# StephenTaf/Modern-Search-Engines-Project

Measured on AMD Instinct MI355X. Metric: queries/sec, two-stage retrieval top-100 (BM25 top-1000 + dense full scan + rerank/fuse), higher is better.
Workload: dtype f32 (exact f32 cosines of every returned document; candidates filtered by one pass of f16 products with a measured margin; batches <= 64 queries: f16x2-split products, |err| <= 8e-6) (dense cosine) / f64 (BM25, fuse)

## Files before the change

modern-search-engines-project_amd/csrc/msr_bm25.hip:

```cpp
#include <stdio.h>

#include "msr_common.h"
#include "msr_internal.h"

namespace {

constexpr int BM25_TILE = MSR_BM25_TILE;
#ifndef BM25_WPW
#define BM25_WPW 1
#endif
constexpr int BM25_WAVES = BM25_WPW;
constexpr int BM25_THREADS = 64 * BM25_WAVES;
constexpr int BM25_TPW = 8;
constexpr int BM25_MAX_TERMS = 64;
constexpr int BM25_CAP = MSR_BM25_ROUND_CAP;
constexpr int BM25_RES = 4;
#ifndef BM25_U
#define BM25_U 4
#endif
#ifndef BM25_UM
#define BM25_UM 8
#endif
constexpr int BM25_WORDS = BM25_TPW * BM25_TILE / 32;
static_assert(BM25_WORDS == 4 * 64, "four bitmap words per lane");
static_assert(BM25_CAP % 128 == 0 && BM25_CAP >= 128 && BM25_CAP <= BM25_TILE, "whole batches of slots; a word (32) always fits");

__device__ __forceinline__ void lds_phase() {
    __builtin_amdgcn_fence(__ATOMIC_ACQ_REL, "wavefront");
    __builtin_amdgcn_wave_barrier();
}

__device__ __forceinline__ int64_t lane_i64(int64_t v, int j) {
    const uint32_t lo = (uint32_t)__builtin_amdgcn_readlane((int)(uint32_t)(uint64_t)v, j);
    const uint32_t hi = (uint32_t)__builtin_amdgcn_readlane((int)(uint32_t)((uint64_t)v >> 32), j);
    return (int64_t)(((uint64_t)hi << 32) | lo);
}
__device__ __forceinline__ double lane_f64(double v, int j) {
    return __longlong_as_double(lane_i64(__double_as_longlong(v), j));
}
__device__ __forceinline__ int lane_rank(unsigned long long m) {
    return (int)__builtin_amdgcn_mbcnt_hi((uint32_t)(m >> 32), __builtin_amdgcn_mbcnt_lo((uint32_t)m, 0u));
}

__device__ __forceinline__ double post_comp(const Bm25Post& x) { return __hiloint2double((int)x.comp_hi, (int)x.comp_lo); }
typedef const __attribute__((address_space(1))) double* gtable;
__device__ __forceinline__ gtable table_of(int64_t bits) { return (gtable)(uint64_t)bits; }

enum : int { K_DEAD = 0, K_LOOKUP = 1, K_HEAVY = 2, K_RANGE = 3 };

#ifndef BM25_WPE
#define BM25_WPE 4
#endif
template <typename... Set>
__global__ __launch_bounds__(BM25_THREADS) __attribute__((amdgpu_waves_per_eu(BM25_WPE, BM25_WPE))) void bm25_taat_kernel(Bm25Index ix,
                                                                  const int32_t* __restrict__ q_term_off,
                                                                  const int32_t* __restrict__ q_terms,
                                                                  const int32_t* __restrict__ q_qtf,
                                                                  int q_first, int nq, double min_score, int tpw, int n_spans,
                                                                  double* __restrict__ cand_score,
                                                                  int32_t* __restrict__ cand_doc,
                                                                  int32_t* __restrict__ seg_n, int dbg_arg, Set... set) {
#ifdef MSR_DIAG
    const int dbg = dbg_arg;
#else
    constexpr int dbg = 0;
#endif
    __shared__ __attribute__((aligned(16))) double acc_all[BM25_WAVES][BM25_CAP];
    __shared__ __attribute__((aligned(16))) uint32_t bits_all[BM25_WAVES][BM25_WORDS];
    __shared__ uint16_t pre_all[BM25_WAVES][BM25_WORDS];
    __shared__ uint16_t slot_all[BM25_WAVES][BM25_CAP];
    const int tid = threadIdx.x, lane = tid & 63;
    const int wave = __builtin_amdgcn_readfirstlane(tid >> 6);
    const int item = (int)blockIdx.x * BM25_WAVES + wave;
    const int span = item / nq, q = item - span * nq;
    if (span >= n_spans) return;
    int32_t* seg_len = seg_n + (int64_t)q * n_spans + span;
    int seg_cnt = 0;
    constexpr bool WITHIN = sizeof...(Set) > 0;
    MsrSetRow srow{nullptr, 0};
    if constexpr (WITHIN) {
        srow = msr_set_row(q_first + q, set...);
        if (srow.mode == 2) {
            if (lane == 0) *seg_len = 0;
            return;
        }
    }
    const int tile0 = span * tpw;
    const int n_my = tile0 + tpw <= ix.n_tiles ? tpw : ix.n_tiles - tile0;
    double* acc = acc_all[wave];
    uint32_t* bits = bits_all[wave];
    uint16_t* pre = pre_all[wave];
    uint16_t* slot = slot_all[wave];
    const int64_t lo_span = (int64_t)tile0 * BM25_TILE;
    const int64_t hi_span = lo_span + (int64_t)n_my * BM25_TILE < ix.n_docs ? lo_span + (int64_t)n_my * BM25_TILE : ix.n_docs;
    const uint32_t n_span = (uint32_t)(hi_span - lo_span);
    const bool prune = min_score >= 0.0 && ix.dense_id != nullptr && !(dbg & 64);
    int nt = 0, klass = K_DEAD;
    int64_t s_v = 0;
    int h_v = -1;
    int64_t ps_v = 0, pe_v = 0;
    double idf_v = 0.0, qtf_v = 0.0;
    bool medium = false;
    {
        const int t0 = q_term_off[q_first + q];
        nt = q_term_off[q_first + q + 1] - t0;
        if (nt > BM25_MAX_TERMS) nt = BM25_MAX_TERMS;
        if (lane < nt) {
            const int32_t t = q_terms[t0 + lane];
            if (t >= 0 && t < ix.n_terms) {
                const int64_t s = ix.term_off[t], e = ix.term_off[t + 1];
                if (e > s) {
                    idf_v = (double)ix.idf[t];
                    qtf_v = (double)q_qtf[t0 + lane];
                    const int dh = prune ? ix.dense_id[t] : -1;
                    const int h = ix.heavy_id ? ix.heavy_id[t] : -1;
                    if (dh >= 0 && idf_v < 0.0 && qtf_v > 0.0) {
                        klass = K_LOOKUP;
                        s_v = (int64_t)(ix.dense_comp + (int64_t)dh * ix.dense_stride);
                    } else if (h >= 0) {
                        klass = K_HEAVY;
                        s_v = s;
                        h_v = h;
                        const uint32_t* row = ix.tile_off + (int64_t)h * (ix.n_tiles + 1) + tile0;
                        ps_v = s + row[0];
                        pe_v = s + row[n_my];
                    } else {
                        klass = K_RANGE;
                        ps_v = s;
                        pe_v = e;
                        medium = e - s > 64;
                    }
                }
            }
        }
    }
    const unsigned long long look_mask = __ballot(klass == K_LOOKUP);
    const unsigned long long stream_mask = __ballot(klass >= K_HEAVY);
    if (stream_mask == 0) {
        if (lane == 0) *seg_len = 0;
        return;
    }
    const int64_t seg_base = (int64_t)q * ix.n_docs + lo_span;
    {
        const int64_t lo8 = lo_span, hi8 = hi_span;
        constexpr int MED = 4;
        unsigned long long todo = __ballot(medium);
        while (todo) {
            int jj[MED];
            int64_t s_[MED], e_[MED], ch_[MED];
            int32_t probe[MED];
#pragma unroll
            for (int m = 0; m < MED; ++m) {
                jj[m] = todo ? __ffsll((long long)todo) - 1 : -1;
                if (todo) todo &= todo - 1;
                probe[m] = 0; s_[m] = e_[m] = ch_[m] = 0;
                if (jj[m] >= 0) {
                    s_[m] = lane_i64(ps_v, jj[m]);
                    e_[m] = lane_i64(pe_v, jj[m]);
                    ch_[m] = (e_[m] - s_[m] + 63) >> 6;
                    int64_t idx = s_[m] + (int64_t)(lane + 1) * ch_[m] - 1;
                    if (idx > e_[m] - 1) idx = e_[m] - 1;
                    probe[m] = ix.post[idx].doc;
                }
            }
#pragma unroll
            for (int m = 0; m < MED; ++m) {
                if (jj[m] < 0) continue;
                const unsigned long long ge_lo = __ballot((int64_t)probe[m] >= lo8);
                const unsigned long long ge_hi = __ballot((int64_t)probe[m] >= hi8);
                int64_t ps = e_[m], pe = e_[m];
                if (ge_lo) {
                    ps = s_[m] + (int64_t)(__ffsll((long long)ge_lo) - 1) * ch_[m];
                    if (ps > e_[m]) ps = e_[m];
                    if (ge_hi) {
                        pe = s_[m] + (int64_t)(__ffsll((long long)ge_hi)) * ch_[m];
                        if (pe > e_[m]) pe = e_[m];
                    }
                }
                if (lane == jj[m]) { ps_v = ps; pe_v = pe; }
            }
        }
    }
    const int64_t null_post = ix.n_postings;
    int cj[BM25_RES];
    int64_t cps[BM25_RES], cpe[BM25_RES];
// ... 320 lines not shown
    }
}

__global__ __launch_bounds__(256) void bm25_dnorm_kernel(const int32_t* __restrict__ doc_len, int64_t n_docs, int64_t n_pad,
                                                          double k1, double b, double avgdl, double* __restrict__ out) {
    const int64_t i = (int64_t)blockIdx.x * 256 + threadIdx.x;
    if (i >= n_pad) return;
    const double omb = 1.0 - b;
    out[i] = i < n_docs ? k1 * (omb + (b * (double)doc_len[i]) / avgdl) : 1.0;
}

int g_bm25_dbg = 0;

}

void msr_bm25_set_dbg(int v) { g_bm25_dbg = v; }
hipError_t msr_bm25_build_skip(const Bm25Index& ix, const int32_t* heavy_terms, int n_heavy, uint32_t* tile_off,
                               hipStream_t stream) {
    if (n_heavy <= 0) return hipSuccess;
    build_skip_kernel<<<n_heavy, 256, 0, stream>>>(ix, heavy_terms, tile_off);
    return hipGetLastError();
}

hipError_t msr_bm25_post_comp(const int32_t* post_doc, const int32_t* post_tf, const double* dnorm, double k1, int64_t n,
                              Bm25Post* out, hipStream_t stream) {
    if (n < 0) return hipSuccess;
    bm25_post_comp_kernel<<<4096, 256, 0, stream>>>(post_doc, post_tf, dnorm, k1 + 1.0, n, out);
    return hipGetLastError();
}

hipError_t msr_bm25_build_dense(const Bm25Index& ix, const int32_t* dense_terms, int n_dense, double* dense_comp,
                                int64_t dense_stride, hipStream_t stream) {
    if (n_dense <= 0) return hipSuccess;
    bm25_dense_kernel<<<dim3(256, (unsigned)n_dense), 256, 0, stream>>>(ix, dense_terms, dense_comp, dense_stride);
    return hipGetLastError();
}

hipError_t msr_bm25_dnorm(const int32_t* doc_len, int64_t n_docs, int64_t n_pad, double k1, double b, double avgdl, double* out,
                          hipStream_t stream) {
    if (n_pad <= 0) return hipSuccess;
    bm25_dnorm_kernel<<<(unsigned)((n_pad + 255) / 256), 256, 0, stream>>>(doc_len, n_docs, n_pad, k1, b, avgdl, out);
    return hipGetLastError();
}

hipError_t msr_bm25_validate(const Bm25Index& ix, int32_t* flag, hipStream_t stream) {
    hipError_t err = hipMemsetAsync(flag, 0x7F, sizeof(int32_t), stream);
    if (err != hipSuccess) return err;
    validate_postings_kernel<<<2048, 256, 0, stream>>>(ix, flag);
    return hipGetLastError();
}

int msr_bm25_max_segments(int64_t n_docs) { return (int)((n_docs + BM25_TILE - 1) / BM25_TILE); }

__global__ __launch_bounds__(256) void bm25_window_kernel(Bm25Index ix, const int32_t* __restrict__ q_term_off,
                                                           const int32_t* __restrict__ q_terms,
                                                           const int32_t* __restrict__ q_qtf, int q_first, int nq,
                                                           uint64_t* __restrict__ out) {
    const int q = blockIdx.x * 256 + threadIdx.x;
    if (q >= nq) return;
    const int t0 = q_term_off[q_first + q];
    int nt = q_term_off[q_first + q + 1] - t0;
    if (nt > BM25_MAX_TERMS) nt = BM25_MAX_TERMS;
    double u = 0.0;
    for (int j = 0; j < nt; ++j) {
        const int32_t t = q_terms[t0 + j];
        if (t < 0 || t >= ix.n_terms) continue;
        const double w = (double)ix.idf[t] * (double)q_qtf[t0 + j];
        if (w > 0.0) u += w;
    }
    u = u * (ix.k1 + 1.0) * 1.0000001 + 1e-300;
    const uint64_t pre = msr_ord64(u) >> 44;
    out[q] = pre > 4094 ? pre - 4094 : 0;
}

hipError_t msr_bm25_window(const Bm25Index& ix, const int32_t* q_term_off, const int32_t* q_terms, const int32_t* q_qtf,
                           int q_first, int nq, uint64_t* out, hipStream_t stream) {
    if (nq <= 0) return hipSuccess;
    bm25_window_kernel<<<(unsigned)((nq + 255) / 256), 256, 0, stream>>>(ix, q_term_off, q_terms, q_qtf, q_first, nq, out);
    return hipGetLastError();
}

void msr_bm25_split(int n_tiles, int nq, int* tpw_out, int* n_spans_out) {
    int tpw = BM25_TPW;
    while (tpw > 1 && (int64_t)nq * ((n_tiles + tpw - 1) / tpw) < 8192) tpw >>= 1;
    *tpw_out = tpw;
    *n_spans_out = (n_tiles + tpw - 1) / tpw;
}

hipError_t msr_bm25_scores(const Bm25Index& ix, const int32_t* q_term_off, const int32_t* q_terms,
                           const int32_t* q_qtf, int q_first, int nq, double min_score, double* cand_score,
                           int32_t* cand_doc, int32_t* seg_n, int* n_seg, int64_t* seg_stride, hipStream_t stream,
                           const MsrSetView* set) {
    *n_seg = 0; *seg_stride = 0;
    if (nq <= 0 || ix.n_docs <= 0) return hipSuccess;
    int tpw = 1, n_spans = 0;
    msr_bm25_split(ix.n_tiles, nq, &tpw, &n_spans);
    const int64_t items = (int64_t)nq * n_spans;
    if (items >= (1ll << 31)) return hipErrorInvalidValue;
    *n_seg = n_spans;
    *seg_stride = (int64_t)tpw * BM25_TILE;
    const unsigned blocks = (unsigned)((items + BM25_WAVES - 1) / BM25_WAVES);
    if (set)
        bm25_taat_kernel<<<blocks, BM25_THREADS, 0, stream>>>(ix, q_term_off, q_terms, q_qtf, q_first, nq, min_score, tpw, n_spans,
                                                              cand_score, cand_doc, seg_n, g_bm25_dbg, *set);
    else
        bm25_taat_kernel<<<blocks, BM25_THREADS, 0, stream>>>(ix, q_term_off, q_terms, q_qtf, q_first, nq, min_score, tpw, n_spans,
                                                              cand_score, cand_doc, seg_n, g_bm25_dbg);
    return hipGetLastError();
}
```

modern-search-engines-project_amd/csrc/msr_engine.hip:

```cpp
#include <hip/hip_runtime.h>
#include <stdarg.h>
#include <stdio.h>
#include <stdlib.h>
#include <string.h>

#include <algorithm>
#include <new>
#include <vector>

#include "../../include/msretr.h"
#include "msr_devmem.h"
#include "msr_internal.h"

struct HipMem {
    static hipError_t alloc(void** p, size_t bytes) { return hipMalloc(p, bytes); }
    static void free(void* p) { (void)hipFree(p); }
};
using Group = DevGroup<HipMem>;

struct msr_engine {
    msr_config cfg;
    char err[512];
    Group mem_engine;
    Group mem_corpus;
    Group mem_postings;
    Group mem_chunks;
    Group mem_bf16;
    Bm25Index bm25{};
    bool have_postings = false;
    const int64_t* tok_off = nullptr;
    const int32_t* tok_ids = nullptr;
    int64_t n_tokens = 0;
    bool have_tokens = false;
    const int64_t* voc_char_off = nullptr;
    const uint16_t* voc_chars = nullptr;
    const uint32_t* voc_weight = nullptr;
    int64_t voc_n_chars = 0;
    bool have_vocab = false;
    FacetTable facet{};
    bool have_facet = false;
    const uint32_t* sig = nullptr;
    int64_t sig_n = 0;
    DenseIndex dense{};
    bool have_chunks = false;
    const int32_t* url_group = nullptr;
    int64_t url_group_n = 0;
    const int32_t* doc_domain = nullptr;
    int64_t doc_domain_n = 0;
    int32_t* chunk_doc = nullptr;
    void* emb_presplit = nullptr;
    void* row_meta = nullptr;
    float* inv_norm_own = nullptr;
    int32_t* span_doc = nullptr;
    int32_t* wspan_doc = nullptr;
    int32_t* wspan12_doc = nullptr;
    float* qn = nullptr;
    float* rr_qn = nullptr;
    void* qimg = nullptr;
    SelScratch sel{};
    float* rerank_cos = nullptr;
    int32_t* rerank_meta = nullptr;
    void* score_rows = nullptr;
    size_t score_rows_bytes = 0;
    int32_t* bm_cand_doc = nullptr;
    size_t bm_cand_bytes = 0;
    int32_t* bm_heavy_id = nullptr;
    void* bm_post = nullptr;
    int32_t* bm_dense_id = nullptr;
    double* bm_dense = nullptr;
    uint32_t* bm_tile_off = nullptr;
    int32_t* bm_cand_n = nullptr;
    uint64_t* bm_win = nullptr;
    uint64_t* voc_sig = nullptr;
    int32_t* bt_top_doc = nullptr; float* bt_top_score = nullptr; int32_t* bt_top_n = nullptr;
    int32_t* bt_cand_doc = nullptr; float* bt_cand_score = nullptr; int32_t* bt_cand_chunk = nullptr;
    int32_t* bt_cand_n = nullptr;
    int32_t* tile_row = nullptr;
    int n_tiles = 0;
    bool tiles_ok = false;
    GemmF32Index gf{};
    bool gf_ok = false;
    float* gf_inv_pad = nullptr; float* gf_qn = nullptr; void* gf_fb_qimg = nullptr;
    int32_t* gf_gate = nullptr;
    void* gf_emb_tiled = nullptr;
    void* gf_emb_f16 = nullptr;
    int32_t* tile_trow = nullptr;
    void* emb_bf16 = nullptr;
    GemmIndex gemm{};
    bool gemm_ok = false;
    float* gm_qn = nullptr;
    uint32_t* bf_err = nullptr;
    float* bf_margin = nullptr;
    float* bf_ones = nullptr;
    void* bf_row_meta = nullptr;
    DenseIndex dense_bf16{};
    int n_cus = 256;
    int split_pending = 0;
    int row_copy_state = 0;
    int row_image_state = 0;
    int last_dense_width = 0;
    int last_dense_segments = 0;
    int32_t* sim_flag = nullptr;
    void* sim_lists = nullptr; size_t sim_lists_bytes = 0;
    void* sim_over = nullptr; size_t sim_over_bytes = 0;
    bool timing = false;
    static constexpr int EV_RING = 256;
    static constexpr int EV_KINDS = 4;
    hipEvent_t ev_start[EV_KINDS][EV_RING] = {};
    hipEvent_t ev_stop[EV_KINDS][EV_RING] = {};
    int ev_count[EV_KINDS] = {0, 0, 0, 0};
};

static constexpr size_t GF_GATE_BYTES = 16 * sizeof(int32_t);

static thread_local char g_create_err[512] = "";

static int fail(msr_engine* e, int code, const char* fmt, ...) {
    char* dst = e ? e->err : g_create_err;
    va_list ap;
    va_start(ap, fmt);
    vsnprintf(dst, 512, fmt, ap);
    va_end(ap);
    return code;
}

// ... 116 lines not shown
    if (cfg->scan_variant != 0 && cfg->scan_variant != 2 && cfg->scan_variant != 7 && cfg->scan_variant != 14 &&
        cfg->scan_variant != 15)
        return fail(nullptr, MSR_ERR_INVALID, "msr_create: scan_variant must be 0, 2, 7, 14 or 15");
    if (cfg->flags & ~(int32_t)(MSR_CFG_NO_ROW_COPY | MSR_CFG_SINGLE_EMIT))
        return fail(nullptr, MSR_ERR_INVALID, "msr_create: unknown flag bits 0x%x", cfg->flags);
    int ndev = 0;
    hipError_t herr = hipGetDeviceCount(&ndev);
    if (herr != hipSuccess || ndev <= 0)
        return fail(nullptr, MSR_ERR_HIP, "msr_create: no HIP device available (%s)",
                    herr == hipSuccess ? "device count is 0" : hipGetErrorString(herr));
    if (cfg->device < 0 || cfg->device >= ndev)
        return fail(nullptr, MSR_ERR_INVALID, "msr_create: device %d out of range (have %d)", cfg->device, ndev);
    msr_engine* e = new (std::nothrow) msr_engine();
    if (!e) return fail(nullptr, MSR_ERR_NOMEM, "msr_create: out of host memory");
    e->cfg = *cfg;
    e->err[0] = 0;
    const int rc = create_scratch(e);
    if (rc) {
        fail(nullptr, rc, "msr_create: %s", e->err);
        msr_destroy(e);
        return rc;
    }
    *out = e;
    return MSR_OK;
}

extern "C" int msr_destroy(msr_engine* e) {
    if (!e) return MSR_OK;
    drop_postings(e);
    drop_chunks(e);
    for (int w = 0; w < msr_engine::EV_KINDS; ++w)
        for (int j = 0; j < msr_engine::EV_RING; ++j) {
            if (e->ev_start[w][j]) (void)hipEventDestroy(e->ev_start[w][j]);
            if (e->ev_stop[w][j]) (void)hipEventDestroy(e->ev_stop[w][j]);
        }
    delete e;
    return MSR_OK;
}

static int ensure_score_rows(msr_engine* e, int64_t n_docs) {
    const size_t pad = (size_t)(n_docs + 31) / 32 * 32;
    const size_t need = std::max((size_t)e->cfg.max_queries * pad * sizeof(double), (size_t)128 * pad * sizeof(float));
    return grow(e, e->mem_corpus, &e->score_rows, &e->score_rows_bytes, need, "score rows");
}

static int build_postings(msr_engine* e, Bm25Index cand, hipStream_t st) {
    const int64_t n_terms = cand.n_terms, n_postings = cand.n_postings, n_docs = cand.n_docs;
    int rc = ensure_score_rows(e, n_docs);
    if (rc) return rc;
    rc = grow(e, e->mem_corpus, &e->bm_cand_doc, &e->bm_cand_bytes, (size_t)e->cfg.max_queries * (size_t)n_docs * sizeof(int32_t),
              "BM25 candidate lists");
    if (rc) return rc;
    ALLOC(e, e->mem_postings, e->bm_win, (size_t)e->cfg.max_queries * sizeof(uint64_t));
    ALLOC(e, e->mem_postings, e->bm_cand_n, (size_t)e->cfg.max_queries * msr_bm25_max_segments(n_docs) * sizeof(int32_t));
    int32_t h_flag = 0;
    HIP_TRY(e, msr_bm25_validate(cand, e->sel.cand_n, st));
    HIP_TRY(e, hipMemcpyAsync(&h_flag, e->sel.cand_n, sizeof(int32_t), hipMemcpyDeviceToHost, st));
    HIP_TRY(e, hipMemsetAsync(e->sel.cand_n, 0, sizeof(int32_t), st));
    HIP_TRY(e, hipStreamSynchronize(st));
    if (h_flag >= 1 && h_flag <= 5) {
        static const char* why[] = {"", "term_off is not a monotone offset array ending at n_postings",
                                    "a posting's document index is outside [0, n_docs)",
                                    "documents are not strictly ascending inside a posting list",
                                    "negative doc_len", "non-positive term frequency"};
        return fail(e, MSR_ERR_INVALID, "msr_bind_postings: malformed index: %s", why[h_flag]);
    }
    if (!(cand.avgdl > 0.0) || !(cand.k1 >= 0.0) || !(cand.b >= 0.0 && cand.b <= 1.0))
        return fail(e, MSR_ERR_INVALID, "msr_bind_postings: avgdl must be > 0, k1 >= 0, 0 <= b <= 1");
    std::vector<int32_t> dense_terms;
    if (n_terms > 0) {
        std::vector<int64_t> h_toff((size_t)n_terms + 1);
        std::vector<float> h_idf((size_t)n_terms);
        HIP_TRY(e, hipMemcpyAsync(h_toff.data(), cand.term_off, h_toff.size() * sizeof(int64_t), hipMemcpyDeviceToHost, st));
        HIP_TRY(e, hipMemcpyAsync(h_idf.data(), cand.idf, h_idf.size() * sizeof(float), hipMemcpyDeviceToHost, st));
        HIP_TRY(e, hipStreamSynchronize(st));
        std::vector<int32_t> heavy_id((size_t)n_terms, -1), heavy_terms;
        for (int64_t t = 0; t < n_terms; ++t)
            if (h_toff[t + 1] - h_toff[t] >= MSR_BM25_HEAVY_DF && h_toff[t + 1] - h_toff[t] < (1ll << 32)) {
                heavy_id[t] = (int32_t)heavy_terms.size();
                heavy_terms.push_back((int32_t)t);
                if (h_idf[t] < 0.0f) dense_terms.push_back((int32_t)t);
            }
        if (!heavy_terms.empty()) {
            DevTemp<HipMem, int32_t> d_terms;
            const size_t rows = heavy_terms.size() * (size_t)(cand.n_tiles + 1);
            ALLOC(e, e->mem_postings, e->bm_heavy_id, heavy_id.size() * sizeof(int32_t));
            ALLOC(e, e->mem_postings, e->bm_tile_off, rows * sizeof(uint32_t));
            ALLOC(e, d_terms.group, d_terms.p, heavy_terms.size() * sizeof(int32_t));
            HIP_TRY(e, hipMemcpyAsync(e->bm_heavy_id, heavy_id.data(), heavy_id.size() * sizeof(int32_t), hipMemcpyHostToDevice, st));
            HIP_TRY(e, hipMemcpyAsync(d_terms.p, heavy_terms.data(), heavy_terms.size() * sizeof(int32_t), hipMemcpyHostToDevice, st));
            HIP_TRY(e, msr_bm25_build_skip(cand, d_terms.p, (int)heavy_terms.size(), e->bm_tile_off, st));
            HIP_TRY(e, hipStreamSynchronize(st));
            cand.heavy_id = e->bm_heavy_id;
            cand.tile_off = e->bm_tile_off;
        }
        std::stable_sort(dense_terms.begin(), dense_terms.end(), [&](int32_t a, int32_t b2) {
            return h_toff[a + 1] - h_toff[a] > h_toff[b2 + 1] - h_toff[b2];
        });
        const size_t row_bytes = ((size_t)cand.n_tiles * MSR_BM25_TILE + 8) * sizeof(double);
        const size_t cap = std::min<size_t>(MSR_BM25_MAX_DENSE, (size_t)(4ull << 30) / row_bytes);
        if (dense_terms.size() > cap) dense_terms.resize(cap);
    }
    {
        const int64_t n_pad = (int64_t)cand.n_tiles * MSR_BM25_TILE;
        DevTemp<HipMem, double> dnorm;
        ALLOC(e, e->mem_postings, e->bm_post, (size_t)(n_postings + 1) * sizeof(Bm25Post));
// ... 418 lines not shown
    if (!e || which < 0 || which >= msr_engine::EV_KINDS || !out_ms) return e ? fail(e, MSR_ERR_INVALID, "msr_kernel_time_ms: bad argument") : MSR_ERR_INVALID;
    const int n = std::min(e->ev_count[which], (int)msr_engine::EV_RING);
    if (n <= 0) return fail(e, MSR_ERR_INVALID, "msr_kernel_time_ms: no timed launch recorded");
    float total = 0.f;
    for (int j = 0; j < n; ++j) {
        float ms = 0.f;
        HIP_TRY(e, hipEventSynchronize(e->ev_stop[which][j]));
        HIP_TRY(e, hipEventElapsedTime(&ms, e->ev_start[which][j], e->ev_stop[which][j]));
        total += ms;
    }
    *out_ms = total;
    if (out_launches) *out_launches = n;
    return MSR_OK;
}

static int within_args_ok(msr_engine* e, const char* fn, int64_t n_docs, const uint32_t* set_bits, int32_t n_sets,
                          int64_t set_stride, const int32_t* q_set) {
    if (n_sets < 0) return fail(e, MSR_ERR_INVALID, "%s: bad argument (n_sets=%d)", fn, n_sets);
    if (n_sets == 0) return MSR_OK;
    if (!set_bits || !q_set) return fail(e, MSR_ERR_INVALID, "%s: bad argument (set_bits or q_set is NULL with n_sets=%d)", fn, n_sets);
    if (set_stride < (n_docs + 31) / 32)
        return fail(e, MSR_ERR_INVALID, "%s: bad argument (set_stride=%lld < ceil(n_docs / 32) = %lld)", fn, (long long)set_stride,
                    (long long)((n_docs + 31) / 32));
    return MSR_OK;
}

static int bm25_topk_impl(msr_engine* e, const char* fn, const int32_t* q_term_off, const int32_t* q_terms, const int32_t* q_qtf,
                          int32_t n_queries, int32_t k, double min_score, int32_t* out_doc, double* out_score, int32_t* out_n,
                          void* stream, const uint32_t* set_bits, int32_t n_sets, int64_t set_stride, const int32_t* q_set) {
    if (!e) return MSR_ERR_INVALID;
    if (!e->have_postings) return fail(e, MSR_ERR_NOT_BOUND, "%s: postings not bound", fn);
    if (n_queries < 0 || k < 1 || k > e->cfg.max_k || !q_term_off || !out_doc || !out_score || !out_n)
        return fail(e, MSR_ERR_INVALID, "%s: bad argument (k=%d, max_k=%d)", fn, k, e->cfg.max_k);
    {
        const int rc = within_args_ok(e, fn, e->bm25.n_docs, set_bits, n_sets, set_stride, q_set);
        if (rc) return rc;
    }
    if (n_queries == 0) return MSR_OK;
    const MsrSetView set_view{set_bits, set_stride, q_set, n_sets};
    const MsrSetView* set = n_sets > 0 ? &set_view : nullptr;
    hipStream_t st = (hipStream_t)stream;
    HIP_TRY(e, hipSetDevice(e->cfg.device));
    const int slice = e->cfg.max_queries;
    const int64_t N = e->bm25.n_docs;
    for (int q0 = 0; q0 < n_queries; q0 += slice) {
        const int nq = std::min(slice, n_queries - q0);
        int32_t* o_doc = out_doc + (int64_t)q0 * k;
        double* o_score = out_score + (int64_t)q0 * k;
        const bool timed = e->timing && e->ev_count[1] < msr_engine::EV_RING;
        int n_seg = 0;
        int64_t seg_stride = 0;
        if (timed) HIP_TRY(e, hipEventRecord(e->ev_start[1][e->ev_count[1]], st));
        HIP_TRY(e, msr_bm25_scores(e->bm25, q_term_off, q_terms, q_qtf, q0, nq, min_score, (double*)e->score_rows, e->bm_cand_doc,
                                   e->bm_cand_n, &n_seg, &seg_stride, st, set));
        if (timed) {
            HIP_TRY(e, hipEventRecord(e->ev_stop[1][e->ev_count[1]], st));
            e->ev_count[1]++;
        }
        const uint64_t* win = nullptr;
        if (min_score >= 0.0) {
            HIP_TRY(e, msr_bm25_window(e->bm25, q_term_off, q_terms, q_qtf, q0, nq, e->bm_win, st));
            win = e->bm_win;
        }
        HIP_TRY(e, msr_select_topk_list((const double*)e->score_rows, e->bm_cand_doc, e->bm_cand_n, n_seg, seg_stride, N, nq, k,
                                        e->sel, o_doc, o_score, out_n + q0, st, win));
    }
    return MSR_OK;
}

extern "C" int msr_bm25_topk(msr_engine* e, const int32_t* q_term_off, const int32_t* q_terms, const int32_t* q_qtf,
                             int32_t n_queries, int32_t k, double min_score, int32_t* out_doc, double* out_score,
                             int32_t* out_n, void* stream) {
    return bm25_topk_impl(e, "msr_bm25_topk", q_term_off, q_terms, q_qtf, n_queries, k, min_score, out_doc, out_score, out_n,
                          stream, nullptr, 0, 0, nullptr);
}

extern "C" int msr_bm25_topk_within(msr_engine* e, const int32_t* q_term_off, const int32_t* q_terms, const int32_t* q_qtf,
                                    int32_t n_queries, int32_t k, double min_score, const uint32_t* set_bits, int32_t n_sets,
                                    int64_t set_stride, const int32_t* q_set, int32_t* out_doc, double* out_score,
                                    int32_t* out_n, void* stream) {
    return bm25_topk_impl(e, "msr_bm25_topk_within", q_term_off, q_terms, q_qtf, n_queries, k, min_score, out_doc, out_score,
                          out_n, stream, set_bits, n_sets, set_stride, q_set);
}

static int tokens_bound(msr_engine* e, const char* fn) {
    if (e->have_postings && e->have_tokens) return MSR_OK;
    return fail(e, MSR_ERR_NOT_BOUND, "%s: tokens not bound (msr_bind_tokens: the index has no forward index)", fn);
}

static int set_rows_args_ok(msr_engine* e, const char* fn, int32_t n_rows, bool rows_ok, const char* rows_what, int64_t out_stride,
                            const char* n_in_name, int32_t n_in, bool in_ok, const char* in_what, const char* in_stride_name,
                            int64_t in_stride) {
    const int64_t W = (e->bm25.n_docs + 31) / 32;
    if (n_rows < 0 || n_in < 0) return fail(e, MSR_ERR_INVALID, "%s: bad argument (n_rows=%d, %s=%d)", fn, n_rows, n_in_name, n_in);
    if (n_rows > 0 && !rows_ok)
        return fail(e, MSR_ERR_INVALID, "%s: bad argument (%s is NULL with n_rows=%d)", fn, rows_what, n_rows);
    if (out_stride < W)
        return fail(e, MSR_ERR_INVALID, "%s: bad argument (out_stride=%lld < ceil(n_docs / 32) = %lld)", fn, (long long)out_stride,
                    (long long)W);
    if (n_in > 0 && !in_ok)
        return fail(e, MSR_ERR_INVALID, "%s: bad argument (%s is NULL with %s=%d)", fn, in_what, n_in_name, n_in);
    if (n_in > 0 && in_stride < W)
        return fail(e, MSR_ERR_INVALID, "%s: bad argument (%s=%lld < ceil(n_docs / 32) = %lld)", fn, in_stride_name,
                    (long long)in_stride, (long long)W);
    return MSR_OK;
}

extern "C" int msr_term_sets(msr_engine* e, int32_t n_rows, const int32_t* must_off, const int32_t* must_terms,
                             const int32_t* not_off, const int32_t* not_terms, const uint32_t* base_bits, int32_t n_base,
                             int64_t base_stride, const int32_t* row_base, uint32_t* out_bits, int64_t out_stride, void* stream) {
    if (!e) return MSR_ERR_INVALID;
    if (!e->have_postings) return fail(e, MSR_ERR_NOT_BOUND, "msr_term_sets: postings not bound");
    const int rc = set_rows_args_ok(e, "msr_term_sets", n_rows, out_bits && must_off && not_off, "out_bits, must_off or not_off",
                                    out_stride, "n_base", n_base, base_bits && row_base, "base_bits or row_base", "base_stride",
                                    base_stride);
    if (rc) return rc;
// ... 1076 lines not shown
```

modern-search-engines-project_amd/csrc/msr_internal.h:

```cpp
#pragma once
#include <hip/hip_runtime.h>
#include <stdint.h>

#define MSR_DIM 768
#define MSR_SEL_BINS 4096
#define MSR_SEL_CAP 4096

struct SelState {
    uint64_t pref_hi, mask_hi;
    uint32_t pref_lo, mask_lo;
    int32_t k_rem;
    int32_t n_above;
    int32_t done;
    int32_t n_sel;
};

struct SelScratch {
    uint32_t* hist;
    SelState* state;
    uint64_t* cand_hi;
    uint32_t* cand_lo;
    int32_t* cand_n;
    const int32_t* gate;
    int gate_per64;
// ... 25 lines not shown
hipError_t msr_select_topk_within(const float* scores, int64_t n, int64_t stride, int nq, int k, const SelScratch& sc,
                                  const MsrSetView& set, int32_t* out_doc, float* out_score, int32_t* out_n, hipStream_t stream);

hipError_t msr_select_topk_list(const double* scores, const int32_t* idx, const int32_t* counts, int n_seg, int64_t seg_stride,
                                int64_t stride, int nq, int k, const SelScratch& sc, int32_t* out_doc,
                                double* out_score, int32_t* out_n, hipStream_t stream, const uint64_t* win_base = nullptr);

hipError_t msr_merge_lists(int score_bits, const int32_t* in_doc, const void* in_score, const int32_t* in_n,
                           const int32_t* in_pay, int n_parts, int64_t part_stride_bytes, int nq, int k, int32_t* out_doc,
                           void* out_score, int32_t* out_n, int32_t* out_pay, hipStream_t stream);

int msr_fail_global(int code, const char* fmt, ...);

constexpr int MSR_SCAN_BLOCK = 4096;
hipError_t exclusive_scan(const int64_t* in, int64_t n, int64_t* out, int64_t* tmp, int64_t* total, hipStream_t st);
inline int64_t exclusive_scan_tmp_words(int64_t n) {
    if (n <= 0) return 0;
    const int64_t nb = (n + MSR_SCAN_BLOCK - 1) / MSR_SCAN_BLOCK, nb2 = (nb + MSR_SCAN_BLOCK - 1) / MSR_SCAN_BLOCK;
    return 2 * nb + 2 * nb2;
}

struct Bm25Post {
    int32_t doc;
    uint32_t comp_lo, comp_hi;
};
struct Bm25Index {
    const int64_t* term_off;
    const int32_t* post_doc;
    const int32_t* post_tf;
    const int32_t* doc_len;
    const float* idf;
    int64_t n_terms, n_postings, n_docs;
    double avgdl, k1, b;
    const int32_t* heavy_id;
    const uint32_t* tile_off;
    int32_t n_tiles;
    const Bm25Post* post;
    const int32_t* dense_id;
    const double* dense_comp;
    int64_t dense_stride;
};
hipError_t msr_bm25_dnorm(const int32_t* doc_len, int64_t n_docs, int64_t n_pad, double k1, double b, double avgdl, double* out,
                          hipStream_t stream);
hipError_t msr_bm25_post_comp(const int32_t* post_doc, const int32_t* post_tf, const double* dnorm, double k1, int64_t n,
                              Bm25Post* out, hipStream_t stream);
hipError_t msr_bm25_build_dense(const Bm25Index& ix, const int32_t* dense_terms, int n_dense, double* dense_comp,
                                int64_t dense_stride, hipStream_t stream);
constexpr int MSR_BM25_TILE = 1024;
constexpr int MSR_BM25_HEAVY_DF = 2048;
constexpr int MSR_BM25_MAX_DENSE = 64;
hipError_t msr_bm25_build_skip(const Bm25Index& ix, const int32_t* heavy_terms, int n_heavy, uint32_t* tile_off,
                               hipStream_t stream);
int msr_bm25_max_segments(int64_t n_docs);
hipError_t msr_bm25_window(const Bm25Index& ix, const int32_t* q_term_off, const int32_t* q_terms, const int32_t* q_qtf,
                           int q_first, int nq, uint64_t* out , hipStream_t stream);
void msr_bm25_split(int n_tiles, int nq, int* tpw, int* n_spans);
hipError_t msr_bm25_scores(const Bm25Index& ix, const int32_t* q_term_off, const int32_t* q_terms,
                           const int32_t* q_qtf, int q_first, int nq, double min_score, double* cand_score,
                           int32_t* cand_doc, int32_t* seg_n, int* n_seg, int64_t* seg_stride, hipStream_t stream,
                           const MsrSetView* set = nullptr);

hipError_t msr_bm25_point(const Bm25Index& ix, const int32_t* q_term_off, const int32_t* q_terms, const int32_t* q_qtf, int nq,
                          const int32_t* doc, const int32_t* doc_n, int max_docs, double* out_score, int32_t* out_touched,
                          hipStream_t stream);
hipError_t msr_union_lists(int nq, const int32_t* lex_doc, const double* lex_score, const int32_t* lex_n, int k_lex,
                           const int32_t* dense_doc, const double* dense_bm25, const int32_t* dense_n, int k_dense,
                           int32_t* out_doc, double* out_score, int32_t* out_src, int32_t* out_n, int max_cand,
                           hipStream_t stream);

hipError_t msr_term_sets_run(const Bm25Index& ix, int n_rows, const int32_t* must_off, const int32_t* must_terms,
                             const int32_t* not_off, const int32_t* not_terms, const uint32_t* base_bits, int n_base,
                             int64_t base_stride, const int32_t* row_base, uint32_t* out_bits, int64_t out_stride,
                             hipStream_t stream);

hipError_t msr_tokens_validate(const int64_t* tok_off, const int32_t* tok_ids, int64_t n_docs, int64_t n_tokens, int64_t n_terms,
                               int32_t* flag, hipStream_t stream);
hipError_t msr_phrase_sets_run(const int64_t* tok_off, const int32_t* tok_ids, int64_t n_docs, int64_t n_terms, int n_rows,
                               const int32_t* phrase_off, const int32_t* phrase_terms, const uint32_t* cand_bits, int n_cand,
                               int64_t cand_stride, const int32_t* row_cand, uint32_t* out_bits, int64_t out_stride,
                               hipStream_t stream);
hipError_t msr_proximity_sets_run(const int64_t* tok_off, const int32_t* tok_ids, int64_t n_docs, int64_t n_terms, int n_rows,
                                  const int32_t* phrase_off, const int32_t* phrase_terms, const int32_t* row_span,
                                  const int32_t* row_ordered, const uint32_t* cand_bits, int n_cand, int64_t cand_stride,
                                  const int32_t* row_cand, uint32_t* out_bits, int64_t out_stride, hipStream_t stream);
hipError_t msr_best_windows_run(const int64_t* tok_off, const int32_t* tok_ids, int64_t n_docs, int64_t n_terms, int n_pairs,
                                const int32_t* pair_doc, const int32_t* pair_row, int n_rows, const int32_t* row_off,
                                const int32_t* row_terms, const int32_t* row_weights, const int32_t* row_span, int32_t* out_start,
                                int32_t* out_cover, int32_t* out_hits, uint64_t* out_mask, uint32_t* out_terms,
                                hipStream_t stream);
hipError_t msr_vocab_validate(const int64_t* char_off, const uint32_t* weight, int64_t n_terms, int64_t n_chars, int32_t* flag,
                              hipStream_t stream);
hipError_t msr_vocab_signatures(const int64_t* char_off, const uint16_t* chars, int64_t n_terms, uint64_t* sig,
                                hipStream_t stream);
int64_t msr_fuzzy_spans(int64_t n_terms);
hipError_t msr_fuzzy_terms_run(const int64_t* char_off, const uint16_t* chars, const uint32_t* weight, const uint64_t* sig,
                               int64_t n_terms, int n_words, const int32_t* word_off, const uint16_t* word_chars,
                               const int32_t* word_max, int limit, int32_t* out_term, int32_t* out_dist, int32_t* out_n,
                               int32_t* out_total, void* scratch, hipStream_t stream);
hipError_t msr_wildcard_terms_run(const int64_t* char_off, const uint16_t* chars, const uint32_t* weight, const uint64_t* sig,
                                  int64_t n_terms, int n_patterns, const int32_t* pat_off, const uint16_t* pat_chars, int limit,
                                  int32_t* out_term, int32_t* out_n, int32_t* out_total, void* scratch, hipStream_t stream);
struct FacetTable {
    const uint16_t* local;
    const int32_t* span_off;
    const int32_t* span_values;
    const int32_t* value_off;
    const int32_t* value_pos;
    int32_t n_values;
    int64_t n_entries;
};
hipError_t msr_facet_validate(const FacetTable& f, int64_t n_docs, int32_t* flag, hipStream_t stream);
int64_t msr_facet_row_bytes(const FacetTable& f, int64_t n_docs);
hipError_t msr_facet_counts_run(const Bm25Index& ix, const FacetTable& f, int n_rows, const int32_t* any_off,
// ... 219 lines not shown
```

Measured before the change: 67880.

## Schedule BM25 work items heaviest-query-first via a planning kernel fused with window

Adds a planning kernel that estimates each query's streamed posting volume, ranks queries by that weight, and writes an order array plus a count of heavy queries. The TAAT kernel then maps work items so heavy queries' spans are dispatched first, to reduce the long-tail imbalance where a few heavy queries finish last. The old per-query window kernel is folded into the planner, saving one launch. The cost is an extra O(nq^2) ranking pass in each block and a cap on batch size (PLAN_MAX).

```diff
diff --git a/modern-search-engines-project_amd/csrc/msr_bm25.hip b/modern-search-engines-project_amd/csrc/msr_bm25.hip
--- a/modern-search-engines-project_amd/csrc/msr_bm25.hip
+++ b/modern-search-engines-project_amd/csrc/msr_bm25.hip
@@ -48,6 +48,31 @@
 
 enum : int { K_DEAD = 0, K_LOOKUP = 1, K_HEAVY = 2, K_RANGE = 3 };
 
+struct Bm25Term {
+    int klass, dh, h;
+    int64_t s, e;
+    double idf, qtf;
+};
+__device__ __forceinline__ Bm25Term bm25_classify(const Bm25Index& ix, int32_t t, int32_t qtf, bool prune) {
+    Bm25Term r{K_DEAD, -1, -1, 0, 0, 0.0, 0.0};
+    if (t < 0 || t >= ix.n_terms) return r;
+    r.s = ix.term_off[t];
+    r.e = ix.term_off[t + 1];
+    const double idf = (double)ix.idf[t];
+    const int dh = prune ? ix.dense_id[t] : -1;
+    const int h = ix.heavy_id ? ix.heavy_id[t] : -1;
+    if (r.e <= r.s) return r;
+    r.idf = idf;
+    r.qtf = (double)qtf;
+    r.dh = dh;
+    r.h = h;
+    r.klass = dh >= 0 && idf < 0.0 && r.qtf > 0.0 ? K_LOOKUP : (h >= 0 ? K_HEAVY : K_RANGE);
+    return r;
+}
+__device__ __forceinline__ bool bm25_prune(const Bm25Index& ix, double min_score) {
+    return min_score >= 0.0 && ix.dense_id != nullptr;
+}
+
 #ifndef BM25_WPE
 #define BM25_WPE 4
 #endif
@@ -59,7 +84,8 @@
                                                                   int q_first, int nq, double min_score, int tpw, int n_spans,
                                                                   double* __restrict__ cand_score,
                                                                   int32_t* __restrict__ cand_doc,
-                                                                  int32_t* __restrict__ seg_n, int dbg_arg, Set... set) {
+                                                                  int32_t* __restrict__ seg_n,
+                                                                  const int32_t* __restrict__ order, int dbg_arg, Set... set) {
 #ifdef MSR_DIAG
     const int dbg = dbg_arg;
 #else
@@ -72,8 +98,18 @@
     const int tid = threadIdx.x, lane = tid & 63;
     const int wave = __builtin_amdgcn_readfirstlane(tid >> 6);
     const int item = (int)blockIdx.x * BM25_WAVES + wave;
-    const int span = item / nq, q = item - span * nq;
-    if (span >= n_spans) return;
+    if (item >= nq * n_spans) return;
+    const int n_heavy = order[nq], heavy_items = n_heavy * n_spans;
+    int span, qj;
+    if (item < heavy_items) {
+        span = item / n_heavy;
+        qj = item - span * n_heavy;
+    } else {
+        const int n_light = nq - n_heavy, r = item - heavy_items;
+        span = r / n_light;
+        qj = n_heavy + (r - span * n_light);
+    }
+    const int q = order[qj];
     int32_t* seg_len = seg_n + (int64_t)q * n_spans + span;
     int seg_cnt = 0;
     constexpr bool WITHIN = sizeof...(Set) > 0;
@@ -94,7 +130,7 @@
     const int64_t lo_span = (int64_t)tile0 * BM25_TILE;
     const int64_t hi_span = lo_span + (int64_t)n_my * BM25_TILE < ix.n_docs ? lo_span + (int64_t)n_my * BM25_TILE : ix.n_docs;
     const uint32_t n_span = (uint32_t)(hi_span - lo_span);
-    const bool prune = min_score >= 0.0 && ix.dense_id != nullptr && !(dbg & 64);
+    const bool prune = bm25_prune(ix, min_score) && !(dbg & 64);
     int nt = 0, klass = K_DEAD;
     int64_t s_v = 0;
     int h_v = -1;
@@ -106,31 +142,22 @@
         nt = q_term_off[q_first + q + 1] - t0;
         if (nt > BM25_MAX_TERMS) nt = BM25_MAX_TERMS;
         if (lane < nt) {
-            const int32_t t = q_terms[t0 + lane];
-            if (t >= 0 && t < ix.n_terms) {
-                const int64_t s = ix.term_off[t], e = ix.term_off[t + 1];
-                if (e > s) {
-                    idf_v = (double)ix.idf[t];
-                    qtf_v = (double)q_qtf[t0 + lane];
-                    const int dh = prune ? ix.dense_id[t] : -1;
-                    const int h = ix.heavy_id ? ix.heavy_id[t] : -1;
-                    if (dh >= 0 && idf_v < 0.0 && qtf_v > 0.0) {
-                        klass = K_LOOKUP;
-                        s_v = (int64_t)(ix.dense_comp + (int64_t)dh * ix.dense_stride);
-                    } else if (h >= 0) {
-                        klass = K_HEAVY;
-                        s_v = s;
-                        h_v = h;
-                        const uint32_t* row = ix.tile_off + (int64_t)h * (ix.n_tiles + 1) + tile0;
-                        ps_v = s + row[0];
-                        pe_v = s + row[n_my];
-                    } else {
-                        klass = K_RANGE;
-                        ps_v = s;
-                        pe_v = e;
-                        medium = e - s > 64;
-                    }
-                }
+            const Bm25Term tm = bm25_classify(ix, q_terms[t0 + lane], q_qtf[t0 + lane], prune);
+            klass = tm.klass;
+            idf_v = tm.idf;
+            qtf_v = tm.qtf;
+            if (klass == K_LOOKUP) {
+                s_v = (int64_t)(ix.dense_comp + (int64_t)tm.dh * ix.dense_stride);
+            } else if (klass == K_HEAVY) {
+                s_v = tm.s;
+                h_v = tm.h;
+                const uint32_t* row = ix.tile_off + (int64_t)tm.h * (ix.n_tiles + 1) + tile0;
+                ps_v = tm.s + row[0];
+                pe_v = tm.s + row[n_my];
+            } else if (klass == K_RANGE) {
+                ps_v = tm.s;
+                pe_v = tm.e;
+                medium = tm.e - tm.s > 64;
             }
         }
     }
@@ -557,32 +584,80 @@
 
 int msr_bm25_max_segments(int64_t n_docs) { return (int)((n_docs + BM25_TILE - 1) / BM25_TILE); }
 
-__global__ __launch_bounds__(256) void bm25_window_kernel(Bm25Index ix, const int32_t* __restrict__ q_term_off,
-                                                           const int32_t* __restrict__ q_terms,
-                                                           const int32_t* __restrict__ q_qtf, int q_first, int nq,
-                                                           uint64_t* __restrict__ out) {
-    const int q = blockIdx.x * 256 + threadIdx.x;
-    if (q >= nq) return;
-    const int t0 = q_term_off[q_first + q];
-    int nt = q_term_off[q_first + q + 1] - t0;
-    if (nt > BM25_MAX_TERMS) nt = BM25_MAX_TERMS;
-    double u = 0.0;
-    for (int j = 0; j < nt; ++j) {
-        const int32_t t = q_terms[t0 + j];
-        if (t < 0 || t >= ix.n_terms) continue;
-        const double w = (double)ix.idf[t] * (double)q_qtf[t0 + j];
-        if (w > 0.0) u += w;
-    }
-    u = u * (ix.k1 + 1.0) * 1.0000001 + 1e-300;
-    const uint64_t pre = msr_ord64(u) >> 44;
-    out[q] = pre > 4094 ? pre - 4094 : 0;
-}
-
-hipError_t msr_bm25_window(const Bm25Index& ix, const int32_t* q_term_off, const int32_t* q_terms, const int32_t* q_qtf,
-                           int q_first, int nq, uint64_t* out, hipStream_t stream) {
-    if (nq <= 0) return hipSuccess;
-    bm25_window_kernel<<<(unsigned)((nq + 255) / 256), 256, 0, stream>>>(ix, q_term_off, q_terms, q_qtf, q_first, nq, out);
-    return hipGetLastError();
+constexpr int PLAN_THREADS = 1024;
+constexpr int PLAN_QUERIES = 64;
+constexpr int PLAN_SLICES = PLAN_THREADS / PLAN_QUERIES;
+constexpr int PLAN_MAX = 4096;
+__global__ __launch_bounds__(PLAN_THREADS) void bm25_plan_kernel(Bm25Index ix, const int32_t* __restrict__ q_term_off,
+                                                                  const int32_t* __restrict__ q_terms,
+                                                                  const int32_t* __restrict__ q_qtf, int q_first, int nq,
+                                                                  double min_score, int tpw, uint64_t* __restrict__ win_out,
+                                                                  int32_t* __restrict__ order) {
+    __shared__ unsigned long long weight[PLAN_MAX];
+    __shared__ int rank_sh[PLAN_QUERIES];
+    __shared__ int n_heavy;
+    const int t = threadIdx.x;
+    const int q_lo = (int)blockIdx.x * PLAN_QUERIES;
+    const bool prune = bm25_prune(ix, min_score);
+    if (t == 0) n_heavy = 0;
+    if (t < PLAN_QUERIES) rank_sh[t] = 0;
+    for (int q = t; q < nq; q += PLAN_THREADS) {
+        const int t0 = q_term_off[q_first + q];
+        int nt = q_term_off[q_first + q + 1] - t0;
+        if (nt > BM25_MAX_TERMS) nt = BM25_MAX_TERMS;
+        double u = 0.0;
+        unsigned long long wt = 0;
+        constexpr int TB = 8;
+        for (int j0 = 0; j0 < nt; j0 += TB) {
+            int32_t tq[TB], tf[TB];
+#pragma unroll
+            for (int j = 0; j < TB; ++j) {
+                tq[j] = j0 + j < nt ? q_terms[t0 + j0 + j] : -1;
+                tf[j] = j0 + j < nt ? q_qtf[t0 + j0 + j] : 0;
+            }
+            Bm25Term tm[TB];
+#pragma unroll
+            for (int j = 0; j < TB; ++j) tm[j] = bm25_classify(ix, tq[j], tf[j], prune);
+#pragma unroll
+            for (int j = 0; j < TB; ++j) {
+                if (tq[j] < 0 || tq[j] >= ix.n_terms) continue;
+                const double w = (double)ix.idf[tq[j]] * (double)tf[j];
+                if (w > 0.0) u += w;
+                if (tm[j].klass >= K_HEAVY) wt += (unsigned long long)(tm[j].e - tm[j].s);
+            }
+        }
+        if (q >= q_lo && q < q_lo + PLAN_QUERIES) {
+            u = u * (ix.k1 + 1.0) * 1.0000001 + 1e-300;
+            const uint64_t pre = msr_ord64(u) >> 44;
+            win_out[q] = pre > 4094 ? pre - 4094 : 0;
+        }
+        weight[q] = wt;
+    }
+    __syncthreads();
+    {
+        const int q = q_lo + (t & (PLAN_QUERIES - 1)), slice = t / PLAN_QUERIES;
+        const int per = (nq + PLAN_SLICES - 1) / PLAN_SLICES;
+        const int o_hi = (slice + 1) * per < nq ? (slice + 1) * per : nq;
+        if (q < nq) {
+            const unsigned long long w = weight[q];
+            int above = 0;
+            for (int o = slice * per; o < o_hi; ++o) {
+                const unsigned long long x = weight[o];
+                above += x > w || (x == w && o < q);
+            }
+            if (above) atomicAdd(&rank_sh[q - q_lo], above);
+        }
+    }
+    __syncthreads();
+    if (t < PLAN_QUERIES && q_lo + t < nq) order[rank_sh[t]] = q_lo + t;
+    if (blockIdx.x != 0) return;
+    const unsigned long long span_docs = (unsigned long long)tpw * BM25_TILE;
+    const unsigned long long heavy_above = (unsigned long long)(BM25_RES * 64) * (unsigned long long)ix.n_docs;
+    int mine_heavy = 0;
+    for (int q = t; q < nq; q += PLAN_THREADS) mine_heavy += weight[q] * span_docs > heavy_above;
+    if (mine_heavy) atomicAdd(&n_heavy, mine_heavy);
+    __syncthreads();
+    if (t == 0) order[nq] = n_heavy;
 }
 
 void msr_bm25_split(int n_tiles, int nq, int* tpw_out, int* n_spans_out) {
@@ -594,22 +669,24 @@
 
 hipError_t msr_bm25_scores(const Bm25Index& ix, const int32_t* q_term_off, const int32_t* q_terms,
                            const int32_t* q_qtf, int q_first, int nq, double min_score, double* cand_score,
-                           int32_t* cand_doc, int32_t* seg_n, int* n_seg, int64_t* seg_stride, hipStream_t stream,
-                           const MsrSetView* set) {
+                           int32_t* cand_doc, int32_t* seg_n, int* n_seg, int64_t* seg_stride, uint64_t* win, int32_t* order,
+                           hipStream_t stream, const MsrSetView* set) {
     *n_seg = 0; *seg_stride = 0;
     if (nq <= 0 || ix.n_docs <= 0) return hipSuccess;
+    if (nq > PLAN_MAX || !win || !order) return hipErrorInvalidValue;
     int tpw = 1, n_spans = 0;
     msr_bm25_split(ix.n_tiles, nq, &tpw, &n_spans);
     const int64_t items = (int64_t)nq * n_spans;
     if (items >= (1ll << 31)) return hipErrorInvalidValue;
     *n_seg = n_spans;
     *seg_stride = (int64_t)tpw * BM25_TILE;
+    bm25_plan_kernel<<<(unsigned)((nq + PLAN_QUERIES - 1) / PLAN_QUERIES), PLAN_THREADS, 0, stream>>>(ix, q_term_off, q_terms, q_qtf, q_first, nq, min_score, tpw, win, order);
     const unsigned blocks = (unsigned)((items + BM25_WAVES - 1) / BM25_WAVES);
     if (set)
         bm25_taat_kernel<<<blocks, BM25_THREADS, 0, stream>>>(ix, q_term_off, q_terms, q_qtf, q_first, nq, min_score, tpw, n_spans,
-                                                              cand_score, cand_doc, seg_n, g_bm25_dbg, *set);
+                                                              cand_score, cand_doc, seg_n, order, g_bm25_dbg, *set);
     else
         bm25_taat_kernel<<<blocks, BM25_THREADS, 0, stream>>>(ix, q_term_off, q_terms, q_qtf, q_first, nq, min_score, tpw, n_spans,
-                                                              cand_score, cand_doc, seg_n, g_bm25_dbg);
+                                                              cand_score, cand_doc, seg_n, order, g_bm25_dbg);
     return hipGetLastError();
 }
diff --git a/modern-search-engines-project_amd/csrc/msr_engine.hip b/modern-search-engines-project_amd/csrc/msr_engine.hip
--- a/modern-search-engines-project_amd/csrc/msr_engine.hip
+++ b/modern-search-engines-project_amd/csrc/msr_engine.hip
@@ -71,6 +71,7 @@
     uint32_t* bm_tile_off = nullptr;
     int32_t* bm_cand_n = nullptr;
     uint64_t* bm_win = nullptr;
+    int32_t* bm_order = nullptr;
     uint64_t* voc_sig = nullptr;
     int32_t* bt_top_doc = nullptr; float* bt_top_score = nullptr; int32_t* bt_top_n = nullptr;
     int32_t* bt_cand_doc = nullptr; float* bt_cand_score = nullptr; int32_t* bt_cand_chunk = nullptr;
@@ -293,6 +294,7 @@
               "BM25 candidate lists");
     if (rc) return rc;
     ALLOC(e, e->mem_postings, e->bm_win, (size_t)e->cfg.max_queries * sizeof(uint64_t));
+    ALLOC(e, e->mem_postings, e->bm_order, ((size_t)e->cfg.max_queries + 1) * sizeof(int32_t));
     ALLOC(e, e->mem_postings, e->bm_cand_n, (size_t)e->cfg.max_queries * msr_bm25_max_segments(n_docs) * sizeof(int32_t));
     int32_t h_flag = 0;
     HIP_TRY(e, msr_bm25_validate(cand, e->sel.cand_n, st));
@@ -817,16 +819,12 @@
         int64_t seg_stride = 0;
         if (timed) HIP_TRY(e, hipEventRecord(e->ev_start[1][e->ev_count[1]], st));
         HIP_TRY(e, msr_bm25_scores(e->bm25, q_term_off, q_terms, q_qtf, q0, nq, min_score, (double*)e->score_rows, e->bm_cand_doc,
-                                   e->bm_cand_n, &n_seg, &seg_stride, st, set));
+                                   e->bm_cand_n, &n_seg, &seg_stride, e->bm_win, e->bm_order, st, set));
         if (timed) {
             HIP_TRY(e, hipEventRecord(e->ev_stop[1][e->ev_count[1]], st));
             e->ev_count[1]++;
         }
-        const uint64_t* win = nullptr;
-        if (min_score >= 0.0) {
-            HIP_TRY(e, msr_bm25_window(e->bm25, q_term_off, q_terms, q_qtf, q0, nq, e->bm_win, st));
-            win = e->bm_win;
-        }
+        const uint64_t* win = min_score >= 0.0 ? e->bm_win : nullptr;
         HIP_TRY(e, msr_select_topk_list((const double*)e->score_rows, e->bm_cand_doc, e->bm_cand_n, n_seg, seg_stride, N, nq, k,
                                         e->sel, o_doc, o_score, out_n + q0, st, win));
     }
diff --git a/modern-search-engines-project_amd/csrc/msr_internal.h b/modern-search-engines-project_amd/csrc/msr_internal.h
--- a/modern-search-engines-project_amd/csrc/msr_internal.h
+++ b/modern-search-engines-project_amd/csrc/msr_internal.h
@@ -101,13 +101,11 @@
 hipError_t msr_bm25_build_skip(const Bm25Index& ix, const int32_t* heavy_terms, int n_heavy, uint32_t* tile_off,
                                hipStream_t stream);
 int msr_bm25_max_segments(int64_t n_docs);
-hipError_t msr_bm25_window(const Bm25Index& ix, const int32_t* q_term_off, const int32_t* q_terms, const int32_t* q_qtf,
-                           int q_first, int nq, uint64_t* out , hipStream_t stream);
 void msr_bm25_split(int n_tiles, int nq, int* tpw, int* n_spans);
 hipError_t msr_bm25_scores(const Bm25Index& ix, const int32_t* q_term_off, const int32_t* q_terms,
                            const int32_t* q_qtf, int q_first, int nq, double min_score, double* cand_score,
-                           int32_t* cand_doc, int32_t* seg_n, int* n_seg, int64_t* seg_stride, hipStream_t stream,
-                           const MsrSetView* set = nullptr);
+                           int32_t* cand_doc, int32_t* seg_n, int* n_seg, int64_t* seg_stride, uint64_t* win, int32_t* order,
+                           hipStream_t stream, const MsrSetView* set = nullptr);
 
 hipError_t msr_bm25_point(const Bm25Index& ix, const int32_t* q_term_off, const int32_t* q_terms, const int32_t* q_qtf, int nq,
                           const int32_t* doc, const int32_t* doc_n, int max_docs, double* out_score, int32_t* out_touched,
```

Result: faster. 70000 (median of 6 runs) (+3.1%).
